# wiedehopf/readsb

Hardware: AMD Instinct MI355X
Metric: IQ Msamples/s demodulated (UC8 2.4 MSps stream, --fix), whole job (higher is better)
Workload: dtype u16

## Files before the change

### readsb_amd/csrc/api.cpp

```cpp
#include "ctx.h"

template <class Pred>
static void stage_wait(mgpu_ctx *c, std::unique_lock<std::mutex> &lk, Pred pred) {
    while (!pred()) {
        if (c->hot.load(std::memory_order_relaxed)) {
            lk.unlock();
            for (int i = 0; i < 32; ++i) __builtin_ia32_pause();
            sched_yield();
            lk.lock();
        } else {
            c->cv.wait(lk);
        }
    }
}

static hipError_t wait_event_spin(hipEvent_t ev) {
    for (unsigned spin = 0;; ++spin) {
        const hipError_t e = hipEventQuery(ev);
        if (e != hipErrorNotReady) return e;
        for (int k = 0; k < 128; ++k) __builtin_ia32_pause();
        if ((spin & 1023) == 1023) sched_yield();
    }
}
static hipError_t wait_stream_spin(hipStream_t s) {
// ... 19 lines not shown
void mgpu_config_defaults(struct mgpu_config *cfg) { config_defaults(cfg); }
void mgpu_config_defaults_abi(struct mgpu_config *cfg, uint32_t struct_bytes, uint32_t abi_version) {
    struct mgpu_config full;
    config_defaults(&full);
    full.abi_version = abi_version;
    std::memcpy(cfg, &full, struct_bytes < sizeof(full) ? struct_bytes : sizeof(full));
}
static void config_defaults(struct mgpu_config *cfg) {
    std::memset(cfg, 0, sizeof(*cfg));
    cfg->device = 0;
    cfg->format = MGPU_FMT_UC8;
    cfg->nfix_crc = 1;
    cfg->fixDF = 1;
    cfg->preamble_threshold = 58;
    cfg->buf_samples = 131072;
    cfg->trailing_samples = kTrailing;
    cfg->max_samples = 64ull * 131072;
    cfg->startup_time_ms = 0;
    cfg->abi_version = MGPU_ABI_VERSION;
}

uint32_t mgpu_abi_version(void) { return MGPU_ABI_VERSION; }

const char *mgpu_strerror(int code) {
    switch (code) {
        case MGPU_OK: return "ok";
        case MGPU_E_INVAL: return "invalid argument or state";
        case MGPU_E_NODEVICE: return "no usable HIP device (libmodes_gpu has no CPU fallback)";
        case MGPU_E_HIP: return "HIP runtime error";
        case MGPU_E_NOMEM: return "out of memory";
        case MGPU_E_OVERFLOW: return "device record pool overflow";
        case MGPU_E_CAPACITY: return "more samples than max_samples";
        case MGPU_E_EOF: return "stream already ended on a short buffer";
        default: return "unknown error";
    }
}

const char *mgpu_last_error(mgpu_ctx *ctx) { return ctx ? ctx->err.c_str() : ""; }

int mgpu_device_count(void) {
    int n = 0;
    if (hipGetDeviceCount(&n) != hipSuccess) return 0;
    return n;
}

static int alloc_slot(mgpu_ctx *c, Slot &sl) {
    const uint64_t n = c->chunk_samples;
    const uint64_t mag_len = (n + kTile - 1) / kTile * kTile + kTile + kHalo + 64;
    HIPCHK(c, hipMalloc(&sl.d_mag, mag_len * sizeof(uint16_t)));
    HIPCHK(c, hipMemsetAsync(sl.d_mag, 0, mag_len * sizeof(uint16_t), c->stream));
    HIPCHK(c, hipMalloc(&sl.d_pool, c->cap_pool * sizeof(PhaseRec)));
    HIPCHK(c, hipMalloc(&sl.d_unit_first, (c->cap_units * (size_t) (kUnit / 2048) + 1) * sizeof(uint32_t)));
    HIPCHK(c, hipMalloc(&sl.d_unit_count, (c->cap_units * (size_t) (kUnit / 2048) + 1) * sizeof(uint32_t)));
    HIPCHK(c, hipMalloc(&sl.d_unit_live, (c->cap_units + 2 + 3 * (c->cap_units / 4 + 2)) * sizeof(uint32_t)));
    sl.class_bytes = (mag_len / 32 + 64 + kUnit / 32) * sizeof(uint32_t);
    HIPCHK(c, hipMalloc(&sl.d_class_final, sl.class_bytes));
    HIPCHK(c, hipMalloc(&sl.d_cand, (c->cap_units * (size_t) kUnit + 64) * sizeof(uint16_t)));
    HIPCHK(c, hipMalloc(&sl.d_cand_count, (c->cap_units * (size_t) (kUnit / kSweepTile) + 1) * sizeof(uint32_t)));
    HIPCHK(c, hipMalloc(&sl.d_dealer, (size_t) 2 * kDealerCounters * kDealerStride * sizeof(uint32_t)));
    HIPCHK(c, hipMemsetAsync(sl.d_dealer, 0, (size_t) 2 * kDealerCounters * kDealerStride * sizeof(uint32_t), c->stream));
    HIPCHK(c, hipMalloc(&sl.d_sweep_part, ((size_t) kSweepGridMax * 4) * sizeof(uint32_t)));
    {
        const size_t nb = c->cap_buffers, words = CNT_NUM + 1 + 4 * nb + kAcLists;
        sl.scratch_bytes = words * sizeof(unsigned long long);
        HIPCHK(c, hipMalloc(&sl.d_scratch, sl.scratch_bytes));
        HIPCHK(c, hipMemsetAsync(sl.d_scratch, 0, sl.scratch_bytes, c->stream));
        HIPCHK(c, hipHostMalloc(&sl.h_scratch, sl.scratch_bytes));
        sl.d_counters = sl.d_scratch;
        sl.d_pool_used = (uint32_t *) (sl.d_scratch + CNT_NUM);
        sl.d_sum_level = sl.d_scratch + CNT_NUM + 1;
        sl.d_sum_power = sl.d_sum_level + nb;
        sl.d_fsum_level = (double *) (sl.d_sum_power + nb);
        sl.d_fsum_power = sl.d_fsum_level + nb;
        sl.h_counters = sl.h_scratch;
        sl.h_sums = sl.h_scratch + CNT_NUM + 1;
        sl.h_fsums = (double *) (sl.h_scratch + CNT_NUM + 1 + 2 * nb);
        if (c->cfg.format != MGPU_FMT_UC8) {
            HIPCHK(c, hipMalloc(&sl.d_fsx, 2 * nb * sizeof(double)));
            HIPCHK(c, hipHostMalloc(&sl.h_fsx, 2 * nb * sizeof(double)));
            HIPCHK(c, hipMemsetAsync(sl.d_fsx, 0, 2 * nb * sizeof(double), c->stream));
            sl.d_fsum_level = sl.d_fsx; sl.d_fsum_power = sl.d_fsx + nb; sl.h_fsums = sl.h_fsx;
        }
    }
    HIPCHK(c, hipMalloc(&sl.d_win, 8 * sizeof(unsigned long long)));
    HIPCHK(c, hipMalloc(&sl.d_win_part, kWinPartWords * sizeof(unsigned long long)));
    HIPCHK(c, hipMalloc(&sl.d_msg_pos, c->cap_msgs * sizeof(uint32_t)));
    HIPCHK(c, hipMalloc(&sl.d_msg_limit, c->cap_msgs * sizeof(uint32_t)));
    HIPCHK(c, hipMalloc(&sl.d_msg_len, c->cap_msgs * sizeof(uint16_t)));
    HIPCHK(c, hipMalloc(&sl.d_msg_skip, c->cap_msgs * sizeof(uint16_t)));
    HIPCHK(c, hipMalloc(&sl.d_msg_sig, c->cap_msgs * sizeof(unsigned long long)));
    {
        const size_t blob = c->cap_msgs * sizeof(Accepted) + c->cap_buffers * sizeof(BufferClock) + 64;
        HIPCHK(c, hipMalloc(&sl.d_blob, blob));
        HIPCHK(c, hipHostMalloc(&sl.h_blob, blob));
    }
    HIPCHK(c, hipMalloc(&sl.d_live, c->cap_pool * sizeof(PhaseRec)));
    HIPCHK(c, hipMalloc(&sl.d_live_sig, c->cap_pool * sizeof(unsigned long long)));
    HIPCHK(c, hipHostMalloc(&sl.h_live, c->cap_pool * sizeof(PhaseRec)));
    HIPCHK(c, hipHostMalloc(&sl.h_live_sig, c->cap_pool * sizeof(unsigned long long)));
    HIPCHK(c, hipEventCreateWithFlags(&sl.ev_window, hipEventDisableTiming));
    HIPCHK(c, hipEventCreateWithFlags(&sl.ev_scan, hipEventDisableTiming));
    HIPCHK(c, hipEventCreateWithFlags(&sl.ev_swept, hipEventDisableTiming));
    HIPCHK(c, hipEventCreateWithFlags(&sl.ev_h2d, hipEventDisableTiming));
    HIPCHK(c, hipEventCreateWithFlags(&sl.ev_pre, hipEventDisableTiming));
    HIPCHK(c, hipEventCreateWithFlags(&sl.ev_fsum, hipEventDisableTiming));
    HIPCHK(c, hipEventCreateWithFlags(&sl.ev_convdone, hipEventDisableTiming));
    HIPCHK(c, hipHostMalloc(&sl.h_win, 8 * sizeof(unsigned long long)));
    HIPCHK(c, hipHostMalloc(&sl.h_sig, c->cap_msgs * sizeof(unsigned long long)));
    HIPCHK(c, hipHostMalloc(&sl.h_msg_pos, c->cap_msgs * sizeof(uint32_t)));
    HIPCHK(c, hipHostMalloc(&sl.h_msg_limit, c->cap_msgs * sizeof(uint32_t)));
    HIPCHK(c, hipHostMalloc(&sl.h_msg_len, c->cap_msgs * sizeof(uint16_t)));
    HIPCHK(c, hipHostMalloc(&sl.h_msg_skip, c->cap_msgs * sizeof(uint16_t)));
    if (c->cfg.mode_ac) {
// ... 406 lines not shown
}

static int enqueue_sweep(mgpu_ctx *c, Slot &sl) {
    const mgpu_config &cfg = c->cfg;
    const uint64_t n = sl.n;
    const uint32_t nunits = (uint32_t) ((n + kUnit - 1) / kUnit);
    hipStream_t s = c->stream;
    SweepParams sp{};
    sp.mag = sl.d_mag; sp.n = n; sp.thr = sl.thr;
    sp.valid_long = c->valid_long; sp.valid_short = c->valid_short;
    sp.fix_df = (cfg.fixDF && cfg.nfix_crc) ? 1 : 0;
    sp.bit_syndrome = c->d_bit_syndrome; sp.parity = c->d_parity; sp.group_syndrome = c->d_group_syndrome;
    sp.tab_long = c->d_tab_long; sp.tab_short = c->d_tab_short; sp.n_long = c->n_long; sp.n_short = c->n_short;
    sp.pool = sl.d_pool; sp.pool_cap = (uint32_t) c->cap_pool; sp.pool_used = sl.d_pool_used;
    sp.unit_first = sl.d_unit_first; sp.unit_count = sl.d_unit_count; sp.nunits = nunits; sp.dealer = sl.d_dealer;
    sp.adder_bitmap = c->d_adder_bitmap; sp.counters = sl.d_counters;
    sp.cand = sl.d_cand; sp.cand_count = sl.d_cand_count; sp.sweep_part = sl.d_sweep_part;
    if (sl.fused_iq) {
        sp.iq = sl.fused_iq; sp.iq_format = (uint32_t) cfg.format; sp.tail = sl.fused_tail; sp.uc8_sym = c->d_uc8_folded + UC8_SYM_OFFSET; sp.mag_w = sl.d_mag;
        sp.sum_level = sl.d_sum_level; sp.sum_power = sl.d_sum_power;
        sp.buf_steps = cfg.buf_samples / (uint32_t) kSweepTile;
    }
#if MGPU_EXPERIMENTS
    sp.debug_stage = c->dbg_stage;
#endif
    {
        sl.sweep_blocks = launch_sweep(sp, s);
        if (sl.timed) HIPCHK(c, hipEventRecord(sl.ev[4], s));
        HIPCHK(c, hipEventRecord(sl.ev_swept, s));
        sl.swept_seq.store(sl.seq, std::memory_order_release);
        if (cfg.format != MGPU_FMT_UC8 && !cfg.mode_ac && !sl.have_mag && sl.fsum_iq) {
            const int rc = enqueue_fsum(c, sl, sl.fsum_iq, sl.ev_swept);
            if (rc != MGPU_OK) return rc;
        }
        sl.slice_blocks = launch_slice(sp, s);
    }
    if (sl.timed) HIPCHK(c, hipEventRecord(sl.ev[2], s));
    return MGPU_OK;
}

static int enqueue_post(mgpu_ctx *c, Slot &sl) {
    const uint64_t n = sl.n;
    const uint32_t nunits = (uint32_t) ((n + kUnit - 1) / kUnit);
    hipStream_t s = c->stream;

    PostSweepParams q{};
    q.pool = sl.d_pool; q.pool_cap = (uint32_t) c->cap_pool; q.variant = c->prescreen_variant; q.unit_first = sl.d_unit_first; q.first_count = sl.d_unit_count; q.nunits = nunits; q.chains_per_unit = (uint32_t) (kUnit / 2048); q.adder_bitmap = c->d_adder_bitmap;
    q.unit_live = sl.d_unit_live; q.block_live = sl.d_unit_live + c->cap_units + 2; q.live = sl.d_live; q.live_sig = sl.d_live_sig; q.counters = sl.d_counters;
    sl.sig_late = (c->sig_late && c->shard_mode == 0) || c->shard_mode == 3;
    q.mag = sl.sig_late ? nullptr : sl.d_mag;
    q.class_final = sl.d_class_final;
    q.class_words = (n + 31) / 32;
    q.dealer = sl.d_dealer;
    q.cand = sl.d_cand; q.cand_count = sl.d_cand_count;
    q.live_win = c->shard_mode == 2 ? sl.d_live_win : nullptr; q.n = n; q.thr = sl.thr; q.buf_len = c->cfg.buf_samples;
    q.d_scratch = sl.d_scratch; q.h_scratch = sl.h_scratch; q.scratch_words = (uint32_t) (sl.scratch_bytes / sizeof(unsigned long long));
    q.fin_part = q.block_live + c->cap_units / 4 + 2;
    q.slice_part = sl.d_sweep_part; q.slice_blocks = sl.slice_blocks;
    if (launch_prescreen(q, s, s, sl.ev_scan) != 0) { c->err = "event ordering of the pre-screen passes failed"; return MGPU_E_HIP; }
    if (sl.timed) HIPCHK(c, hipEventRecord(sl.ev[3], s));
    HIPCHK(c, hipEventRecord(sl.ev_done, s));
    return MGPU_OK;
}

static int enqueue_slot(mgpu_ctx *c, Slot &sl, const uint8_t *iq, hipEvent_t after_convert = nullptr) {
    int rc = enqueue_convert(c, sl, iq);
    const bool fsum_late = (c->cfg.format != MGPU_FMT_UC8 && !c->cfg.mode_ac && !sl.have_mag) || sweep_is_fused(c, sl);
    auto mark_read = [&]() -> int {
        if (sl.fsum_pending) {
            HIPCHK(c, hipEventRecord(sl.ev_convdone, c->stream));
            HIPCHK(c, hipStreamWaitEvent(c->stream_f, sl.ev_convdone, 0));
            HIPCHK(c, hipEventRecord(after_convert, c->stream_f));
        } else HIPCHK(c, hipEventRecord(after_convert, c->stream));
        return MGPU_OK;
    };
    if (rc == MGPU_OK && after_convert && !fsum_late) rc = mark_read();
    if (rc == MGPU_OK) rc = enqueue_sweep(c, sl);
    if (rc == MGPU_OK && after_convert && fsum_late) rc = mark_read();
    if (rc == MGPU_OK) rc = enqueue_post(c, sl);
    return rc;
}

static void unpin_records(mgpu_ctx *c, Slot &sl, HostJob &job, bool team) {
    const uint64_t nlive = job.nlive;
    job.recs.resize(nlive + 1);
    job.recs[nlive].pos = 0xFFFFFFFFu;
    if (!sl.sig_late) job.sig.resize(nlive);
    const int parts = team && nlive >= 65536 ? c->walk_threads : 1;
    auto copy = [&](int i) {
        const uint64_t lo = nlive * (uint64_t) i / parts, hi = nlive * (uint64_t) (i + 1) / parts;
        std::memcpy(job.recs.data() + lo, sl.h_live + lo, (hi - lo) * sizeof(PhaseRec));
        if (!sl.sig_late) std::memcpy(job.sig.data() + lo, sl.h_live_sig + lo, (hi - lo) * sizeof(unsigned long long));
    };
    if (parts > 1) c->walk_team.run(parts, copy); else copy(0);
    if (c->shard_mode == 2) job.win.assign(sl.h_live_win, sl.h_live_win + nlive);
    job.fetched = true;
}

static int fetch_records(mgpu_ctx *c, Slot &sl, HostJob &job) {
    const uint64_t nlive = job.nlive;
    if (nlive) {
        HIPCHK(c, hipMemcpyAsync(sl.h_live, sl.d_live, nlive * sizeof(PhaseRec), hipMemcpyDeviceToHost, c->stream_d2h));
        if (!sl.sig_late) HIPCHK(c, hipMemcpyAsync(sl.h_live_sig, sl.d_live_sig, nlive * sizeof(unsigned long long), hipMemcpyDeviceToHost, c->stream_d2h));
        if (c->shard_mode == 2) HIPCHK(c, hipMemcpyAsync(sl.h_live_win, sl.d_live_win, nlive * sizeof(unsigned long long), hipMemcpyDeviceToHost, c->stream_d2h));
        HIPCHK(c, wait_stream_spin(c->stream_d2h));
    }
    if (!c->dump_dir.empty()) {
        const char *dd = c->dump_dir.c_str();
        static int dumped = 0;
        if (!dumped++) {
            std::string base = std::string(dd) + "/walk_";
            FILE *f = fopen((base + "recs.bin").c_str(), "wb"); fwrite(sl.h_live, sizeof(PhaseRec), nlive, f); fclose(f);
            f = fopen((base + "sig.bin").c_str(), "wb"); fwrite(sl.h_live_sig, 8, nlive, f); fclose(f);
            f = fopen((base + "bufs.bin").c_str(), "wb"); fwrite(sl.buffers.data(), sizeof(BufferClock), sl.buffers.size(), f); fclose(f);
        }
    }
    unpin_records(c, sl, job, false);
    return MGPU_OK;
}

static int fetch_slot(mgpu_ctx *c, Slot &sl, HostJob &job) {
    HIPCHK(c, wait_event_spin(sl.ev_done));
    const double t_gpu_done = wall_ms();
    if (sl.h_counters[CNT_POOL_OVERFLOW]) {
        c->err = "record pool overflow: recreate the context with a larger record_pool_records";
        return MGPU_E_OVERFLOW;
    }
    float ms;
    if (sl.timed) {
        if (!sl.fused_iq && hipEventElapsedTime(&ms, sl.ev[0], sl.ev[1]) == hipSuccess) c->acc.convert_ms += ms;
        if (hipEventElapsedTime(&ms, sl.ev[1], sl.ev[4]) == hipSuccess) { c->acc.sweep_ms += ms; sweep_pace_feedback(ms * 1e3f, sl.n, sl.sweep_blocks, c->event_bracket_us, !sl.fused_iq ? 0 : c->cfg.format == MGPU_FMT_UC8 ? 1 : 2); }
        if (hipEventElapsedTime(&ms, sl.ev[4], sl.ev[2]) == hipSuccess) c->acc.slice_ms += ms;
        if (hipEventElapsedTime(&ms, sl.ev[2], sl.ev[3]) == hipSuccess) c->acc.prescreen_ms += ms;
        c->acc.n_timed_chunks += 1;
        if (sl.fused_iq) c->acc.sweep_fused_chunks += 1.0f;
    }
    const uint64_t nlive = sl.h_counters[CNT_LIVE_TOTAL];

    const double t_f0 = wall_ms();
    if (nlive > c->cap_pool) { c->err = "live record count beyond the pool"; return MGPU_E_OVERFLOW; }
    job.nlive = nlive;
    job.stream_pos = sl.stream_pos;
    job.fetched = job.from_device = false;
    job.sig_late = sl.sig_late;
    if ((c->device_walk != 1 || c->shard_mode != 0) && c->shard_mode != 1) { const int rc = fetch_records(c, sl, job); if (rc != MGPU_OK) return rc; }
    job.ac.clear();
    if (c->cfg.mode_ac && (!sl.have_mag || sl.have_noise)) {
        const unsigned long long *counts = sl.h_scratch + CNT_NUM + 1 + 4 * c->cap_buffers;
        const uint64_t cap_l = c->cap_ac / kAcLists;
        for (int l = 0; l < kAcLists; ++l) {
            if (counts[l] > cap_l) { c->err = "Mode A/C candidate buffer overflow"; return MGPU_E_OVERFLOW; }
            job.ac.insert(job.ac.end(), sl.h_ac + (size_t) l * cap_l, sl.h_ac + (size_t) l * cap_l + counts[l]);
        }
    }
    job.buffers = sl.buffers;
    job.given_mean_power = sl.given_mean_power;
    job.sums.assign(sl.h_sums, sl.h_sums + 2 * c->cap_buffers);
    job.fsum_idx = -1;
    if (sl.fsum_pending) {
        sl.fsum_pending = false;
        if (c->shard_mode == 0) job.fsum_idx = sl.fsum_idx;
        else {
            HIPCHK(c, wait_event_spin(c->fsum_ring[sl.fsum_idx].ev));
            std::memcpy(sl.h_fsums, c->fsum_ring[sl.fsum_idx].h, 2 * c->cap_buffers * sizeof(double));
        }
    }
    if (job.fsum_idx < 0) job.fsums.assign(sl.h_fsums, sl.h_fsums + 2 * c->cap_buffers);
    const unsigned long long *hc = sl.h_counters;
    if (!(c->shard_stream && job.stream_pos < c->shard_stream_own_first)) {
        c->feed_cand[0] += hc[CNT_CANDIDATES];
        for (int i = 0; i < 5; ++i) c->feed_cand[1 + i] += hc[CNT_PHASE0 + i];
        c->feed_cand[6] += hc[CNT_CLASS_COND];
        c->feed_cand[7] += hc[CNT_CLASS_UNCOND];
    }
    c->acc.n_candidates += hc[CNT_CANDIDATES];
    c->acc.n_records += hc[CNT_RECORDS];
    c->acc.n_live_records += nlive;
    c->acc.n_chunks += 1;
    c->acc.d2h_ms += (float) (wall_ms() - t_f0);
// ... 1152 lines not shown
```

### readsb_amd/csrc/ctx.h

```cpp
#pragma once
#include <hip/hip_runtime.h>
#include <pthread.h>
#include <dirent.h>
#include <sched.h>

#include <cctype>
#include <algorithm>
#include <atomic>
#include <functional>
#include <chrono>
#include <condition_variable>
#include <deque>
#include <mutex>
#include <thread>
#include <cmath>
#include <cstdio>
#include <cstdlib>
#include <cstring>
#include <limits>
#include <new>
#include <string>
#include <vector>

#include "../../include/modes_gpu.h"
// ... 56 lines not shown
  private:
    void work(uint32_t g, const std::function<void(int)> *fn, int n) {
        int done = 0;
        uint64_t t = ticket_.load(std::memory_order_acquire);
        for (;;) {
            if ((uint32_t) (t >> 32) != g || (int) (uint32_t) t >= n) break;
            if (!ticket_.compare_exchange_weak(t, t + 1, std::memory_order_acq_rel)) continue;
            (*fn)((int) (uint32_t) t);
            ++done;
            t = ticket_.load(std::memory_order_acquire);
        }
        if (done && pending_.fetch_sub(done, std::memory_order_acq_rel) == done) {
            std::lock_guard<std::mutex> lk(mu_);
            cv_done_.notify_all();
        }
    }
    void loop() {
        uint64_t seen = wake_.load(std::memory_order_acquire);
        for (;;) {
            for (int spin = 0; wake_.load(std::memory_order_acquire) == seen; ++spin) {
                __builtin_ia32_pause();
                if ((spin & 63) == 63) sched_yield();
                if (spin >= 4000 && !(hot_ && hot_->load(std::memory_order_relaxed))) break;
            }
            const std::function<void(int)> *fn;
            int n;
            uint32_t g;
            {
                std::unique_lock<std::mutex> lk(mu_);
                cv_work_.wait(lk, [&] { return quit_ || wake_.load(std::memory_order_acquire) != seen; });
                if (quit_) return;
                seen = wake_.load(std::memory_order_acquire);
                fn = fn_; n = ntasks_; g = gen_;
            }
            if (fn) work(g, fn, n);
        }
    }
    std::mutex mu_;
    std::condition_variable cv_work_, cv_done_;
    const std::function<void(int)> *fn_ = nullptr;
    int ntasks_ = 0;
    uint32_t gen_ = 0;
    std::atomic<uint64_t> ticket_{0}, wake_{0};
    std::atomic<int> pending_{0};
    const std::atomic<bool> *hot_ = nullptr;
    bool quit_ = false;
};

struct Slot {
    uint16_t *d_mag = nullptr;
    PhaseRec *d_pool = nullptr;
    uint32_t *d_dealer = nullptr;
    uint32_t *d_pool_used = nullptr, *d_unit_first = nullptr, *d_unit_count = nullptr, *d_unit_live = nullptr;
    uint32_t *d_class_final = nullptr, *d_cand_count = nullptr, *d_sweep_part = nullptr;
    uint16_t *d_cand = nullptr;
    size_t class_bytes = 0;
    unsigned long long *d_scratch = nullptr, *h_scratch = nullptr;
    size_t scratch_bytes = 0;
    unsigned long long *d_counters = nullptr, *d_sum_level = nullptr, *d_sum_power = nullptr, *d_win = nullptr, *d_msg_sig = nullptr;
    unsigned long long *d_win_part = nullptr;
    double *d_fsum_level = nullptr, *d_fsum_power = nullptr;
    uint32_t *d_msg_pos = nullptr, *d_msg_limit = nullptr;
    uint16_t *d_msg_len = nullptr, *d_msg_skip = nullptr;
    PhaseRec *d_live = nullptr;
    unsigned long long *d_live_sig = nullptr;
    unsigned long long *d_live_win = nullptr, *h_live_win = nullptr;
    PhaseRec *h_live = nullptr;
    unsigned long long *h_live_sig = nullptr;
    hipEvent_t ev_window = nullptr;
    bool window_pending = false;
    unsigned long long *h_counters = nullptr, *h_sums = nullptr, *h_win = nullptr, *h_sig = nullptr;
    double *h_fsums = nullptr;
    double *d_fsx = nullptr, *h_fsx = nullptr;
    uint32_t *h_msg_pos = nullptr, *h_msg_limit = nullptr;
    uint16_t *h_msg_len = nullptr, *h_msg_skip = nullptr;
    hipEvent_t ev_done = nullptr;
    hipEvent_t ev[5] = {};
    bool timed = false;
    uint32_t slice_blocks = 0;
    uint32_t sweep_blocks = 0;
    uint32_t *d_ac_noise = nullptr;
    AcCand *h_ac = nullptr;
    hipEvent_t ev_h2d = nullptr;
    hipEvent_t ev_pre = nullptr, ev_fsum = nullptr, ev_convdone = nullptr;
    bool fsum_pending = false;
    const uint8_t *fsum_iq = nullptr;
    int fsum_idx = -1;
    hipEvent_t ev_scan = nullptr;
    hipEvent_t ev_swept = nullptr;
    std::atomic<uint64_t> swept_seq{~0ull};
    const uint8_t *fused_iq = nullptr;
    const uint16_t *fused_tail = nullptr;
    uint64_t seq = 0;
    uint64_t n = 0, stream_pos = 0;
    uint8_t *d_wk_in = nullptr;
    void *d_wk_acc = nullptr;
    unsigned long long *d_wk_sig = nullptr;
    uint8_t *h_blob = nullptr, *d_blob = nullptr;
    bool sig_late = false;
    int feed = -1;
    int32_t thr = 58;
    bool have_mag = false, busy = false;
    bool have_noise = false;
    uint32_t given_noise = 0;
    std::vector<BufferClock> buffers;
    std::vector<double> given_mean_power;
// ... 228 lines not shown
```

### readsb_amd/csrc/kernels.h

```cpp
#pragma once
#ifndef MGPU_EXPERIMENTS
#define MGPU_EXPERIMENTS 0
#endif
#include <hip/hip_runtime.h>
#include <cstdint>

#include "../../include/modes_gpu.h"

namespace mgpu {

constexpr int kWinPartWords = 8192 * 8;
constexpr int kTrailing = 326;
constexpr int kTile = 4096;
constexpr int kHalo = 304;
constexpr int kTilesPerUnit = 2;
constexpr int kUnit = kTile * kTilesPerUnit;
constexpr int kBlock = 256;
constexpr int kSweepTile = 1024;
#ifndef MGPU_SL_WGS_PER_CU
#define MGPU_SL_WGS_PER_CU 4
#endif
constexpr int kSweepMaxBlocks = 256 * MGPU_SL_WGS_PER_CU;
constexpr int kSweepGridMax = 256 * 8;
constexpr int kDealerCounters = 64;
constexpr int kDealerStride = 64;
constexpr int kPoolChunkRecords = 256;
constexpr int kSweepMaxWaves = kSweepMaxBlocks * (kBlock / 64);
constexpr uint32_t kNone = 0xFFFFFFFFu;

enum : uint8_t {
    REC_ACCEPT_IF_UNKNOWN = 1,
    REC_ADDER = 2,
    REC_DFFIX = 4,
    REC_LONG = 8,
    REC_CORR_SHIFT = 4,
    REC_COND = 64,
};

struct PhaseRec {
    uint32_t pos;
    uint8_t phase;
    uint8_t flags;
    int16_t score_known;
    int16_t score_unknown;
    uint8_t fixbit0, fixbit1;
    uint32_t addr;
    uint8_t msg[14];
    uint16_t pad;
};
static_assert(sizeof(PhaseRec) == 32, "PhaseRec must be 32 bytes");
static_assert(sizeof(mgpu_msg) == 64 && sizeof(mgpu_fields) == 176, "C-ABI record sizes");

enum {
    CNT_CANDIDATES = 0,
    CNT_PHASE0 = 1,
    CNT_RECORDS = 6,
    CNT_POOL_OVERFLOW = 7,
    CNT_CLASS_COND = 8,
    CNT_CLASS_UNCOND = 9,
    CNT_DEBUG0 = 16,
    CNT_LIVE_TOTAL = 31,
    CNT_NUM = 32,
};

struct SweepParams {
    const uint16_t *mag;
    uint64_t n;
    int32_t thr;
    uint32_t valid_long;
    uint32_t valid_short;
    int32_t fix_df;
    const uint32_t *bit_syndrome;
    const uint64_t *parity;
    const uint32_t *group_syndrome;
    const uint64_t *tab_long;
    const uint64_t *tab_short;
    int32_t n_long, n_short;
    PhaseRec *pool;
    uint32_t pool_cap;
    uint32_t *pool_used;
    uint32_t *unit_first;
    uint32_t *unit_count;
    uint32_t *dealer;
    uint32_t nunits;
    uint16_t *cand;
    uint32_t *cand_count;
    uint32_t pace_recip;
    uint32_t *sweep_part;
    uint32_t *adder_bitmap;
    unsigned long long *counters;
    const uint8_t *iq;
    uint32_t iq_format;
    const uint16_t *tail;
    const uint16_t *uc8_sym;
    uint16_t *mag_w;
    unsigned long long *sum_level, *sum_power;
    uint32_t buf_steps;
#if MGPU_EXPERIMENTS
    int32_t debug_stage;
    unsigned long long *dbg_waves;
#endif
};

struct ConvertParams {
    const uint8_t *iq;
    uint16_t *mag;
    uint64_t n;
    uint32_t buf_samples;
    const uint16_t *tail;
    const uint16_t *uc8_folded;
    unsigned long long *sum_level;
    unsigned long long *sum_power;
    double *fsum_level;
    double *fsum_power;
};

void launch_convert(int format, const ConvertParams &p, hipStream_t s);
void launch_spin(unsigned us, unsigned blocks, unsigned long long *sink, hipStream_t s);
void launch_fsum_sc16(int format, const uint8_t *iq, uint64_t n, uint32_t buf_samples, double *fsum_level, double *fsum_power, int want_level,
                      hipStream_t s, int fresh = 0);
#if MGPU_EXPERIMENTS
size_t fsum_wide_scratch_bytes(uint64_t max_samples, uint32_t buf_samples);
void launch_fsum_sc16_wide(int format, const uint8_t *iq, const uint16_t *mag, uint64_t n, uint32_t buf_samples, double *fsum_level, double *fsum_power,
                           int want_level, void *scratch, hipStream_t s);
#endif
unsigned launch_sweep(const SweepParams &p, hipStream_t s);
void sweep_pace_feedback(float kernel_us, uint64_t n, unsigned blocks, float bracket_us, int fused = 0);
unsigned launch_slice(const SweepParams &p, hipStream_t s);
struct PostSweepParams {
    PhaseRec *pool;
    uint32_t pool_cap;
    uint32_t variant;
    const uint32_t *unit_first;
    const uint32_t *first_count;
    uint32_t chains_per_unit;
    uint32_t nunits;
    const uint32_t *adder_bitmap;
    uint32_t *unit_live;
    uint32_t *block_live;
    PhaseRec *live;
    const uint16_t *mag;
    unsigned long long *live_sig;
    unsigned long long *counters;
    uint32_t *class_final;
    uint64_t class_words;
    uint32_t *dealer;
    const uint16_t *cand; const uint32_t *cand_count;
    unsigned long long *live_win;
    uint64_t n; int32_t thr; uint32_t buf_len;
    unsigned long long *d_scratch, *h_scratch;
    uint32_t scratch_words;
    uint32_t *fin_part;
    const uint32_t *slice_part;
    uint32_t slice_blocks;
};
int launch_prescreen(const PostSweepParams &q, hipStream_t s, hipStream_t s_write, hipEvent_t ev_scan);
constexpr int kAcLists = 64;
struct AcCand {
    uint32_t pos;
    uint32_t f2_clock;
    uint32_t modeac;
};
void launch_modeac(const uint16_t *mag, uint64_t n, uint32_t buf_samples, int format, const unsigned long long *sum_level,
                   const unsigned long long *sum_power, const double *fsum_level, const double *fsum_power,
                   uint32_t *noise_level, AcCand *out, uint32_t cap, unsigned long long *list_counts ,
                   unsigned long long *counters, hipStream_t s);
void launch_modeac_scan(const uint16_t *mag, uint64_t n, uint32_t buf_samples, const uint32_t *noise_level, AcCand *out, uint32_t cap,
                        unsigned long long *list_counts, unsigned long long *counters, hipStream_t s);
void launch_decode_fields(const mgpu_msg *msgs, uint64_t n, mgpu_fields *out, const double *roll_tan, hipStream_t s);
void launch_beast_encode(const mgpu_msg *msgs, uint64_t n, uint16_t *meta, uint32_t *block_bytes, unsigned long long *block_off, uint8_t *out,
                         uint64_t cap, unsigned long long *total , hipStream_t s, const uint8_t *verdict = nullptr, int net_rule = 0,
                         uint32_t *block_def = nullptr, unsigned long long *block_def_off = nullptr, mgpu_deferred *deferred = nullptr, uint64_t def_cap = 0);
size_t gate_table_bytes();
size_t gate_scratch_bytes(uint64_t n);
void launch_track_gate(const mgpu_msg *msgs, const mgpu_fields *fields, uint64_t n, uint32_t buf_samples, void *table, void *scratch,
                       uint8_t *verdict, hipStream_t s);
void launch_signal_power(const uint16_t *mag, const uint32_t *pos, const uint16_t *len, uint32_t nmsg,
                         unsigned long long *out, hipStream_t s);
void launch_build_messages(const PhaseRec *live, const unsigned long long *live_sig, const unsigned long long *msg_sig, const void *d_acc,
                           const void *d_bufs, uint32_t nacc, mgpu_msg *out, hipStream_t s);
void launch_stage_blob(const void *h_src, void *d_dst, uint64_t bytes, hipStream_t s);

constexpr uint32_t kWkNoAdd = 0xffffffffu;
constexpr uint32_t kWkTouchedCap = 1u << 16;
constexpr int kWkCounts = 16;
constexpr int32_t kWkNoFlip = 0x7fffffff;
struct WalkIn {
    int64_t next_flip;
    uint32_t nbuf, n_active, n_inactive, acc_cap;
    uint32_t nlive, buf_len, pad[2];
};
static_assert(sizeof(WalkIn) == 40, "WalkIn");
constexpr uint32_t kWkInHead = 48;
struct WalkState {
    int32_t flip;
    uint32_t converged, iterations, bad;
    uint32_t n_touched[2];
    uint32_t cur, done;
};
// ... 34 lines not shown
```

### readsb_amd/csrc/kernels/prescreen.inc

```


__device__ __forceinline__ uint32_t write_unit_sequential(uint32_t u, const PhaseRec *pool, const uint32_t *unit_first, uint32_t cpu, uint32_t nunits,
                                                          uint32_t dst0, PhaseRec *live, const uint16_t *mag, unsigned long long *live_sig) {
    const int lane = lane_id();
    if (u >= nunits) return 0;
    uint32_t nlive = 0;
    uint32_t heads = kNone;
    if ((uint32_t) lane < cpu) heads = unit_first[u * cpu + (uint32_t) lane];
    for (uint32_t ch = 0; ch < cpu; ++ch) {
        uint32_t h = (uint32_t) __builtin_amdgcn_readlane((int) heads, (int) ch);
        while (h != kNone) {
            const uint32_t next = pool[h].addr;
            const uint64_t m = ((const unsigned long long *) &pool[h])[2];
            const bool ok = (m >> lane) & 1;
            uint32_t pos = 0, len = 0;
            if (ok) {
                const PhaseRec &r = pool[h + 1 + (uint32_t) lane];
                pos = r.pos;
                len = (r.msg[0] & 0x80) ? 268u : 134u;
                const uint32_t d = dst0 + nlive + __popcll(m & ((1ull << lane) - 1));
                const u32x4 *src = (const u32x4 *) &r;
                u32x4 *dd = (u32x4 *) &live[d];
                dd[0] = src[0]; dd[1] = src[1];
            }
// ... 143 lines not shown
            first = false;
            const uint32_t t0 = (uint32_t) __builtin_amdgcn_readlane((int) hd1.w, 0);
            base1 = base0 + t0;
            total = t0;
            if (CPU == 4) {
                const uint32_t t1 = (uint32_t) __builtin_amdgcn_readlane((int) hd1.w, 1), t2 = (uint32_t) __builtin_amdgcn_readlane((int) hd1.w, 2),
                               t3 = (uint32_t) __builtin_amdgcn_readlane((int) hd1.w, 3);
                base2 = base1 + t1; base3 = base2 + t2;
                total = t0 + t1 + t2 + t3;
            }
        }
#define MGPU_WR_LOAD(ch, base) \
        const uint32_t hc##ch = (uint32_t) __builtin_amdgcn_readlane((int) h, ch); \
        const uint64_t m##ch = (uint64_t) (uint32_t) __builtin_amdgcn_readlane((int) hd1.x, ch) | ((uint64_t) (uint32_t) __builtin_amdgcn_readlane((int) hd1.y, ch) << 32); \
        const bool ok##ch = hc##ch != kNone && ((m##ch >> lane) & 1); \
        const uint32_t d##ch = (base) + (uint32_t) __builtin_amdgcn_readlane((int) hd1.z, ch) + (uint32_t) __popcll(m##ch & lt_mask); \
        u32x4 a##ch = {0u, 0u, 0u, 0u}, b##ch = {0u, 0u, 0u, 0u}; \
        if (ok##ch) { const u32x4 *src = (const u32x4 *) &pool[hc##ch + 1u + (uint32_t) lane]; a##ch = src[0]; b##ch = src[1]; }
#define MGPU_WR_STORE(ch) \
        if (ok##ch) { u32x4 *dd = (u32x4 *) &live[d##ch]; dd[0] = a##ch; dd[1] = b##ch; }
        MGPU_WR_LOAD(0, base0)
        if (CPU == 4) {
            MGPU_WR_LOAD(1, base1) MGPU_WR_LOAD(2, base2) MGPU_WR_LOAD(3, base3)
            MGPU_WR_STORE(0) MGPU_WR_STORE(1) MGPU_WR_STORE(2) MGPU_WR_STORE(3)
        } else {
            MGPU_WR_STORE(0)
        }
#undef MGPU_WR_LOAD
#undef MGPU_WR_STORE
        WAVE_SYNC();
        if (h != kNone) h = hd0.w;
    }
    return total;
}

__global__ __launch_bounds__(kBlock) void k_count(PhaseRec *pool, uint32_t pool_cap, const uint32_t *unit_first, const uint32_t *first_count, uint32_t cpu, uint32_t nunits,
                                                  const uint32_t *bitmap, uint32_t *unit_live, uint32_t *block_live, uint32_t *final_bitmap,
                                                  unsigned long long *counters, uint32_t *part) {
    __shared__ uint32_t s_live[kBlock / WAVE], s_nc[kBlock / WAVE], s_nu[kBlock / WAVE];
    __shared__ __attribute__((aligned(16))) uint32_t s_cls[kBlock / WAVE][2 * (kUnit / 32)];
    const uint32_t wv = threadIdx.x >> 6, u = blockIdx.x * (kBlock / WAVE) + wv;
    uint32_t nlive, nc, nu;
    if (cpu == 4) nlive = count_unit_chains<4>(u, pool, pool_cap, unit_first, first_count, nunits, bitmap, counters, s_cls[wv], final_bitmap, nc, nu);
    else nlive = count_unit_chains<1>(u, pool, pool_cap, unit_first, nullptr, nunits, bitmap, counters, s_cls[wv], final_bitmap, nc, nu);
    if (lane_id() == 0) { s_live[wv] = nlive; s_nc[wv] = nc; s_nu[wv] = nu; if (u < nunits) unit_live[u] = nlive; }
    __syncthreads();
    if (threadIdx.x == 0) {
        block_live[blockIdx.x] = s_live[0] + s_live[1] + s_live[2] + s_live[3];
        part[2 * blockIdx.x] = s_nc[0] + s_nc[1] + s_nc[2] + s_nc[3];
        part[2 * blockIdx.x + 1] = s_nu[0] + s_nu[1] + s_nu[2] + s_nu[3];
    }
}

template <bool SIG>
__global__ __launch_bounds__(kBlock) void k_prescreen_write(PhaseRec *pool, const uint32_t *unit_first, uint32_t cpu, uint32_t nunits,
                                                            int by_chains, const uint32_t *unit_live, const uint32_t *block_live,
                                                            PhaseRec *live, const uint16_t *mag, unsigned long long *live_sig,
                                                            unsigned long long *counters, const uint32_t *fin_part, uint32_t nb_fin,
                                                            const uint32_t *slice_part, uint32_t slice_blocks) {
    __shared__ uint32_t s_part[kBlock / WAVE];
    if (blockIdx.x == 0 && slice_blocks) {
        unsigned long long a[5] = {0, 0, 0, 0, 0};
        for (uint32_t r = threadIdx.x; r < slice_blocks; r += kBlock) {
#pragma unroll
            for (int k = 0; k < 5; ++k) a[k] += slice_part[r * kSlPartWords + k];
        }
#pragma unroll
        for (int k = 0; k < 5; ++k) a[k] = wave_sum_u64(a[k]);
        if (lane_id() == 0) {
            if (a[0]) atomicAdd(&counters[CNT_RECORDS], a[0]);
            if (a[1]) atomicAdd(&counters[CNT_CANDIDATES], a[1]);
            if (a[2]) { atomicAdd(&counters[CNT_PHASE0 + 0], a[2]); atomicAdd(&counters[CNT_PHASE0 + 1], a[2]); }
            if (a[3]) { atomicAdd(&counters[CNT_PHASE0 + 2], a[3]); atomicAdd(&counters[CNT_PHASE0 + 3], a[3]); }
            if (a[4]) atomicAdd(&counters[CNT_PHASE0 + 4], a[4]);
        }
    }
    if (blockIdx.x == 0 && nb_fin) {
        unsigned long long a = 0, b = 0;
        for (uint32_t i = threadIdx.x; i < nb_fin; i += kBlock) { a += fin_part[2 * i]; b += fin_part[2 * i + 1]; }
        a = wave_sum_u64(a); b = wave_sum_u64(b);
        if (lane_id() == 0) {
            if (a) atomicAdd(&counters[CNT_CLASS_COND], a);
            if (b) atomicAdd(&counters[CNT_CLASS_UNCOND], b);
        }
    }
    uint32_t acc = 0;
    for (uint32_t i = threadIdx.x; i < blockIdx.x; i += kBlock) acc += block_live[i];
    acc = (uint32_t) wave_sum_u64(acc);
    const uint32_t wv = threadIdx.x >> 6;
    if (lane_id() == 0) s_part[wv] = acc;
    __syncthreads();
    uint32_t dst0 = s_part[0] + s_part[1] + s_part[2] + s_part[3];
    const uint32_t u = blockIdx.x * (kBlock / WAVE) + wv;
    for (uint32_t v = blockIdx.x * (kBlock / WAVE); v < u && v < nunits; ++v) dst0 += unit_live[v];
    uint32_t nlive;
    if (!SIG && by_chains && cpu == 4) nlive = write_unit_chains<4>(u, pool, unit_first, nunits, dst0, live);
    else if (!SIG && by_chains) nlive = write_unit_chains<1>(u, pool, unit_first, nunits, dst0, live);
    else nlive = write_unit_sequential(u, pool, unit_first, cpu, nunits, dst0, live, SIG ? mag : nullptr, SIG ? live_sig : nullptr);
    if (u == nunits - 1 && lane_id() == 0) counters[CNT_LIVE_TOTAL] = dst0 + nlive;
}

__global__ __launch_bounds__(kBlock) void k_publish(unsigned long long *d_scratch, unsigned long long *h_scratch, uint32_t nwords, uint32_t *dealer) {
    if (blockIdx.x == 0 && dealer && threadIdx.x < 2 * kDealerCounters) dealer[threadIdx.x * kDealerStride] = 0;
    for (uint32_t i = blockIdx.x * kBlock + threadIdx.x; i < nwords; i += gridDim.x * kBlock) {
        h_scratch[i] = d_scratch[i];
        d_scratch[i] = 0;
    }
}

#if MGPU_EXPERIMENTS
__global__ __launch_bounds__(kBlock) void k_prescreen_check(const PhaseRec *pool, const uint32_t *unit_first, uint32_t cpu, uint32_t nunits, const uint32_t *unit_live, unsigned long long *counters) {
    const uint32_t u = blockIdx.x * kBlock + threadIdx.x;
    if (u >= nunits) return;
    uint32_t all = 0;
    for (uint32_t ch = 0; ch < cpu; ++ch) {
        uint32_t h = unit_first[u * cpu + ch], run = 0, seg = 0;
        const uint32_t h0 = h;
        while (h != kNone) {
            const uint32_t *hw = (const uint32_t *) &pool[h];
            const uint64_t m = (uint64_t) hw[4] | ((uint64_t) hw[5] << 32);
            if (hw[6] != run && atomicAdd(&counters[CNT_DEBUG0], 1ull) < 8)
                printf("check: unit %u chain %u segment %u header %u: prefix %u, expected %u (cnt %u mask %llx next %u)\n", u, ch, seg, h, hw[6], run, hw[0], (unsigned long long) m, hw[3]);
            if (hw[0] < 64 && (m >> hw[0]) && atomicAdd(&counters[CNT_DEBUG0], 1ull) < 8)
                printf("check: unit %u chain %u segment %u header %u: mask %llx beyond cnt %u\n", u, ch, seg, h, (unsigned long long) m, hw[0]);
            run += (uint32_t) __popcll(m);
            h = hw[3];
            ++seg;
        }
        if (h0 != kNone && ((const uint32_t *) &pool[h0])[7] != run && atomicAdd(&counters[CNT_DEBUG0], 1ull) < 8)
            printf("check: unit %u chain %u first header %u: total %u, expected %u (%u segments)\n", u, ch, h0, ((const uint32_t *) &pool[h0])[7], run, seg);
        all += run;
    }
    if (all != unit_live[u] && atomicAdd(&counters[CNT_DEBUG0], 1ull) < 8) printf("check: unit %u: live %u, chains add up to %u\n", u, unit_live[u], all);
}
#endif

#if MGPU_EXPERIMENTS
__global__ __launch_bounds__(kBlock) void k_prescreen_check_live(const PhaseRec *pool, const uint32_t *unit_first, uint32_t cpu, uint32_t nunits, const uint32_t *unit_live, const PhaseRec *live, unsigned long long *counters) {
    const uint32_t u = blockIdx.x * kBlock + threadIdx.x;
    if (u >= nunits) return;
    uint32_t d = 0;
    for (uint32_t v = 0; v < u; ++v) d += unit_live[v];
    if (u == 0) printf("live: checked %u units\n", nunits);
    for (uint32_t ch = 0; ch < cpu; ++ch) {
        uint32_t h = unit_first[u * cpu + ch], seg = 0;
        while (h != kNone) {
            const uint32_t *hw = (const uint32_t *) &pool[h];
            const uint64_t m = (uint64_t) hw[4] | ((uint64_t) hw[5] << 32);
            for (uint32_t i = 0; i < hw[0]; ++i) {
                if (!((m >> i) & 1)) continue;
                const uint32_t *a = (const uint32_t *) &pool[h + 1 + i], *b = (const uint32_t *) &live[d];
                bool same = true;
                for (int k = 0; k < 8; ++k) same = same && a[k] == b[k];
                if (!same && atomicAdd(&counters[CNT_DEBUG0 + 1], 1ull) < 12)
                    printf("live: unit %u chain %u segment %u header %u record %u of %u -> live[%u]: pos %u addr %06x, found pos %u addr %06x (mask %llx prefix %u total7 %u)\n",
                           u, ch, seg, h, i, hw[0], d, a[0], a[3], b[0], b[3], (unsigned long long) m, hw[6], hw[7]);
                ++d;
            }
            h = hw[3];
            ++seg;
        }
    }
}
#endif

int launch_prescreen(const PostSweepParams &q, hipStream_t s, hipStream_t s_write, hipEvent_t ev_scan) {
    if (q.nunits == 0) return 0;
    if (q.chains_per_unit != 4 && q.chains_per_unit != 1) return -1;
    const unsigned nb_count = (q.nunits + 3) / 4;
    const unsigned nb_fin = nb_count;
    hipLaunchKernelGGL(k_count, dim3(nb_count), dim3(kBlock), 0, s, q.pool, q.pool_cap, q.unit_first, q.first_count, q.chains_per_unit, q.nunits, q.adder_bitmap,
                       q.unit_live, q.block_live, q.class_final, q.counters, q.fin_part);
#if MGPU_EXPERIMENTS
    if (q.variant & 4) hipLaunchKernelGGL(k_prescreen_check, dim3((q.nunits + kBlock - 1) / kBlock), dim3(kBlock), 0, s, q.pool, q.unit_first, q.chains_per_unit, q.nunits, q.unit_live, q.counters);
#endif
    if (s_write != s) {
        if (hipEventRecord(ev_scan, s) != hipSuccess || hipStreamWaitEvent(s_write, ev_scan, 0) != hipSuccess) return -1;
    }
#define MGPU_WRITE_ARGS dim3(nb_count), dim3(kBlock), 0, s_write, q.pool, q.unit_first, q.chains_per_unit, q.nunits, (q.variant & 2) ? 1 : 0, \
                        q.unit_live, q.block_live, q.live, q.mag, q.live_sig, q.counters, q.fin_part, nb_fin, q.slice_part, q.slice_blocks
    if (q.mag) hipLaunchKernelGGL((k_prescreen_write<true>), MGPU_WRITE_ARGS);
    else hipLaunchKernelGGL((k_prescreen_write<false>), MGPU_WRITE_ARGS);
#undef MGPU_WRITE_ARGS
#if MGPU_EXPERIMENTS
    if (q.variant & 4) hipLaunchKernelGGL(k_prescreen_check_live, dim3((q.nunits + kBlock - 1) / kBlock), dim3(kBlock), 0, s_write, q.pool, q.unit_first, q.chains_per_unit, q.nunits, q.unit_live, q.live, q.counters);
#endif
    if (q.live_win)
        launch_live_windows(q.mag, q.n, q.cand, q.cand_count, q.class_final, q.live, q.counters + CNT_LIVE_TOTAL, q.buf_len, q.live_win, s_write);
    unsigned pb = (q.scratch_words + kBlock - 1) / kBlock;
    if (pb > 64) pb = 64;
    hipLaunchKernelGGL(k_publish, dim3(pb), dim3(kBlock), 0, s_write, q.d_scratch, q.h_scratch, q.scratch_words, q.dealer);
    return 0;
}
```

Before: 462,400.

## Fuse prescreen count and write into one persistent kernel with decoupled look-back scan

Adds a persistent k_prescreen_fused kernel that hands out tickets of units from a dealer counter, counts live records per unit, and computes output offsets with a decoupled look-back prefix scan. It then writes the live records in the same kernel, replacing the separate k_count and k_prescreen_write launches. The goal is to cut one launch and the global round trip of per-unit counts. It adds epoch-tagged look-back state, a stall counter and an error path. The path only runs when prescreen variant bit 8 is set, which may not be the default.

After: 439,100. 0.95x the previous value.

```diff
diff --git a/readsb_amd/csrc/api.cpp b/readsb_amd/csrc/api.cpp
--- a/readsb_amd/csrc/api.cpp
+++ b/readsb_amd/csrc/api.cpp
@@ -95,13 +95,15 @@
     HIPCHK(c, hipMalloc(&sl.d_pool, c->cap_pool * sizeof(PhaseRec)));
     HIPCHK(c, hipMalloc(&sl.d_unit_first, (c->cap_units * (size_t) (kUnit / 2048) + 1) * sizeof(uint32_t)));
     HIPCHK(c, hipMalloc(&sl.d_unit_count, (c->cap_units * (size_t) (kUnit / 2048) + 1) * sizeof(uint32_t)));
-    HIPCHK(c, hipMalloc(&sl.d_unit_live, (c->cap_units + 2 + 3 * (c->cap_units / 4 + 2)) * sizeof(uint32_t)));
+    sl.lookback_at = (c->cap_units + 2 + 3 * (c->cap_units / 4 + 2) + 1) / 2 * 2;
+    HIPCHK(c, hipMalloc(&sl.d_unit_live, (sl.lookback_at + 8 * (c->cap_units / 4 + 2)) * sizeof(uint32_t)));
+    HIPCHK(c, hipMemsetAsync(sl.d_unit_live, 0, (sl.lookback_at + 8 * (c->cap_units / 4 + 2)) * sizeof(uint32_t), c->stream));
     sl.class_bytes = (mag_len / 32 + 64 + kUnit / 32) * sizeof(uint32_t);
     HIPCHK(c, hipMalloc(&sl.d_class_final, sl.class_bytes));
     HIPCHK(c, hipMalloc(&sl.d_cand, (c->cap_units * (size_t) kUnit + 64) * sizeof(uint16_t)));
     HIPCHK(c, hipMalloc(&sl.d_cand_count, (c->cap_units * (size_t) (kUnit / kSweepTile) + 1) * sizeof(uint32_t)));
-    HIPCHK(c, hipMalloc(&sl.d_dealer, (size_t) 2 * kDealerCounters * kDealerStride * sizeof(uint32_t)));
-    HIPCHK(c, hipMemsetAsync(sl.d_dealer, 0, (size_t) 2 * kDealerCounters * kDealerStride * sizeof(uint32_t), c->stream));
+    HIPCHK(c, hipMalloc(&sl.d_dealer, (size_t) kDealerWords * sizeof(uint32_t)));
+    HIPCHK(c, hipMemsetAsync(sl.d_dealer, 0, (size_t) kDealerWords * sizeof(uint32_t), c->stream));
     HIPCHK(c, hipMalloc(&sl.d_sweep_part, ((size_t) kSweepGridMax * 4) * sizeof(uint32_t)));
     {
         const size_t nb = c->cap_buffers, words = CNT_NUM + 1 + 4 * nb + kAcLists;
@@ -614,6 +616,12 @@
     q.class_final = sl.d_class_final;
     q.class_words = (n + 31) / 32;
     q.dealer = sl.d_dealer;
+    q.lookback = (unsigned long long *) (sl.d_unit_live + sl.lookback_at);
+    if (++sl.prescreen_epoch >= (1u << 30)) {
+        HIPCHK(c, hipMemsetAsync(q.lookback, 0, (size_t) 4 * (c->cap_units / 4 + 2) * sizeof(unsigned long long), s));
+        sl.prescreen_epoch = 1;
+    }
+    q.epoch = sl.prescreen_epoch;
     q.cand = sl.d_cand; q.cand_count = sl.d_cand_count;
     q.live_win = c->shard_mode == 2 ? sl.d_live_win : nullptr; q.n = n; q.thr = sl.thr; q.buf_len = c->cfg.buf_samples;
     q.d_scratch = sl.d_scratch; q.h_scratch = sl.h_scratch; q.scratch_words = (uint32_t) (sl.scratch_bytes / sizeof(unsigned long long));
@@ -687,6 +695,10 @@
     if (sl.h_counters[CNT_POOL_OVERFLOW]) {
         c->err = "record pool overflow: recreate the context with a larger record_pool_records";
         return MGPU_E_OVERFLOW;
+    }
+    if (sl.h_counters[CNT_PRESCREEN_STALL]) {
+        c->err = "the pre-screen's look-back gave up waiting for an earlier ticket";
+        return MGPU_E_HIP;
     }
     float ms;
     if (sl.timed) {
diff --git a/readsb_amd/csrc/ctx.h b/readsb_amd/csrc/ctx.h
--- a/readsb_amd/csrc/ctx.h
+++ b/readsb_amd/csrc/ctx.h
@@ -132,6 +132,8 @@
     PhaseRec *d_pool = nullptr;
     uint32_t *d_dealer = nullptr;
     uint32_t *d_pool_used = nullptr, *d_unit_first = nullptr, *d_unit_count = nullptr, *d_unit_live = nullptr;
+    size_t lookback_at = 0;
+    uint32_t prescreen_epoch = 0;
     uint32_t *d_class_final = nullptr, *d_cand_count = nullptr, *d_sweep_part = nullptr;
     uint16_t *d_cand = nullptr;
     size_t class_bytes = 0;
diff --git a/readsb_amd/csrc/kernels.h b/readsb_amd/csrc/kernels.h
--- a/readsb_amd/csrc/kernels.h
+++ b/readsb_amd/csrc/kernels.h
@@ -24,6 +24,12 @@
 constexpr int kSweepGridMax = 256 * 8;
 constexpr int kDealerCounters = 64;
 constexpr int kDealerStride = 64;
+constexpr int kDealerWords = (2 * kDealerCounters + 1) * kDealerStride;
+#ifndef MGPU_FUSED_BATCH
+#define MGPU_FUSED_BATCH 4
+#endif
+constexpr int kFusedBatch = MGPU_FUSED_BATCH;
+constexpr int kFusedTicketUnits = kFusedBatch * (kBlock / 64);
 constexpr int kPoolChunkRecords = 256;
 constexpr int kSweepMaxWaves = kSweepMaxBlocks * (kBlock / 64);
 constexpr uint32_t kNone = 0xFFFFFFFFu;
@@ -58,6 +64,7 @@
     CNT_POOL_OVERFLOW = 7,
     CNT_CLASS_COND = 8,
     CNT_CLASS_UNCOND = 9,
+    CNT_PRESCREEN_STALL = 10,
     CNT_DEBUG0 = 16,
     CNT_LIVE_TOTAL = 31,
     CNT_NUM = 32,
@@ -145,6 +152,8 @@
     uint32_t *class_final;
     uint64_t class_words;
     uint32_t *dealer;
+    unsigned long long *lookback;
+    uint32_t epoch;
     const uint16_t *cand; const uint32_t *cand_count;
     unsigned long long *live_win;
     uint64_t n; int32_t thr; uint32_t buf_len;
diff --git a/readsb_amd/csrc/kernels/prescreen.inc b/readsb_amd/csrc/kernels/prescreen.inc
--- a/readsb_amd/csrc/kernels/prescreen.inc
+++ b/readsb_amd/csrc/kernels/prescreen.inc
@@ -219,6 +219,23 @@
     }
 }
 
+__device__ __forceinline__ void fold_slice_part(const uint32_t *slice_part, uint32_t slice_blocks, unsigned long long *counters) {
+    unsigned long long a[5] = {0, 0, 0, 0, 0};
+    for (uint32_t r = threadIdx.x; r < slice_blocks; r += kBlock) {
+#pragma unroll
+        for (int k = 0; k < 5; ++k) a[k] += slice_part[r * kSlPartWords + k];
+    }
+#pragma unroll
+    for (int k = 0; k < 5; ++k) a[k] = wave_sum_u64(a[k]);
+    if (lane_id() == 0) {
+        if (a[0]) atomicAdd(&counters[CNT_RECORDS], a[0]);
+        if (a[1]) atomicAdd(&counters[CNT_CANDIDATES], a[1]);
+        if (a[2]) { atomicAdd(&counters[CNT_PHASE0 + 0], a[2]); atomicAdd(&counters[CNT_PHASE0 + 1], a[2]); }
+        if (a[3]) { atomicAdd(&counters[CNT_PHASE0 + 2], a[3]); atomicAdd(&counters[CNT_PHASE0 + 3], a[3]); }
+        if (a[4]) atomicAdd(&counters[CNT_PHASE0 + 4], a[4]);
+    }
+}
+
 template <bool SIG>
 __global__ __launch_bounds__(kBlock) void k_prescreen_write(PhaseRec *pool, const uint32_t *unit_first, uint32_t cpu, uint32_t nunits,
                                                             int by_chains, const uint32_t *unit_live, const uint32_t *block_live,
@@ -226,22 +243,7 @@
                                                             unsigned long long *counters, const uint32_t *fin_part, uint32_t nb_fin,
                                                             const uint32_t *slice_part, uint32_t slice_blocks) {
     __shared__ uint32_t s_part[kBlock / WAVE];
-    if (blockIdx.x == 0 && slice_blocks) {
-        unsigned long long a[5] = {0, 0, 0, 0, 0};
-        for (uint32_t r = threadIdx.x; r < slice_blocks; r += kBlock) {
-#pragma unroll
-            for (int k = 0; k < 5; ++k) a[k] += slice_part[r * kSlPartWords + k];
-        }
-#pragma unroll
-        for (int k = 0; k < 5; ++k) a[k] = wave_sum_u64(a[k]);
-        if (lane_id() == 0) {
-            if (a[0]) atomicAdd(&counters[CNT_RECORDS], a[0]);
-            if (a[1]) atomicAdd(&counters[CNT_CANDIDATES], a[1]);
-            if (a[2]) { atomicAdd(&counters[CNT_PHASE0 + 0], a[2]); atomicAdd(&counters[CNT_PHASE0 + 1], a[2]); }
-            if (a[3]) { atomicAdd(&counters[CNT_PHASE0 + 2], a[3]); atomicAdd(&counters[CNT_PHASE0 + 3], a[3]); }
-            if (a[4]) atomicAdd(&counters[CNT_PHASE0 + 4], a[4]);
-        }
-    }
+    if (blockIdx.x == 0 && slice_blocks) fold_slice_part(slice_part, slice_blocks, counters);
     if (blockIdx.x == 0 && nb_fin) {
         unsigned long long a = 0, b = 0;
         for (uint32_t i = threadIdx.x; i < nb_fin; i += kBlock) { a += fin_part[2 * i]; b += fin_part[2 * i + 1]; }
@@ -267,8 +269,140 @@
     if (u == nunits - 1 && lane_id() == 0) counters[CNT_LIVE_TOTAL] = dst0 + nlive;
 }
 
+constexpr uint32_t kLbAggregate = 1, kLbInclusive = 2, kLbFailed = 3;
+constexpr uint32_t kLbMaxPolls = 1u << 15;
+constexpr int kLbWindows = 4;
+constexpr int kLbStride = 4;
+
+__device__ __forceinline__ unsigned long long lb_word(uint32_t epoch, uint32_t status, uint32_t value) {
+    return ((unsigned long long) epoch << 34) | ((unsigned long long) status << 32) | value;
+}
+
+__device__ __forceinline__ bool lookback_exclusive(const unsigned long long *lb, uint32_t t, uint32_t epoch, uint32_t &excl) {
+    const int lane = lane_id();
+    int hi = (int) t;
+    uint32_t sum = 0, polls = 0;
+    while (hi > 0) {
+        unsigned long long w[kLbWindows];
+#pragma unroll
+        for (int k = 0; k < kLbWindows; ++k) {
+            const int i = hi - 1 - k * WAVE - lane;
+            w[k] = i >= 0 ? __hip_atomic_load(&lb[(size_t) kLbStride * (size_t) i], __ATOMIC_RELAXED, __HIP_MEMORY_SCOPE_AGENT) : 0ull;
+        }
+        bool done = false, stuck = false;
+#pragma unroll
+        for (int k = 0; k < kLbWindows; ++k) {
+            if (done || stuck || hi <= 0) continue;
+            const bool in = hi - 1 - lane >= 0;
+            const uint32_t st = (in && (uint32_t) (w[k] >> 34) == epoch) ? (uint32_t) (w[k] >> 32) & 3u : 0u;
+            const uint64_t need = __ballot(in), ready = __ballot(st != 0), inc = __ballot(st == kLbInclusive), bad = __ballot(st == kLbFailed);
+            if (bad) return false;
+            const uint64_t upto = inc ? (((inc & (0 - inc)) << 1) - 1) & need : need;
+            if ((ready & upto) != upto) { stuck = true; continue; }
+            sum += (uint32_t) wave_sum_u64(((upto >> lane) & 1) ? (uint32_t) w[k] : 0u);
+            if (inc) done = true; else hi -= WAVE;
+        }
+        if (done) break;
+        if (stuck) {
+            if (++polls > kLbMaxPolls) return false;
+            __builtin_amdgcn_s_sleep(2);
+        }
+    }
+    excl = sum;
+    return true;
+}
+
+__global__ __launch_bounds__(kBlock, 5) void k_prescreen_fused(PhaseRec *pool, uint32_t pool_cap, const uint32_t *unit_first, const uint32_t *first_count, uint32_t nunits,
+                                                               const uint32_t *bitmap, uint32_t *unit_live, uint32_t *final_bitmap, PhaseRec *live,
+                                                               unsigned long long *counters, const uint32_t *slice_part, uint32_t slice_blocks,
+                                                               uint32_t *ticket_counter, unsigned long long *lb, uint32_t epoch) {
+    constexpr int kWaves = kBlock / WAVE, kB = kFusedBatch;
+    static_assert(kWaves == 4, "a group = four units, one per wave");
+    __shared__ uint32_t s_live[kB][kWaves], s_nc[kWaves], s_nu[kWaves], s_ticket, s_excl, s_fail;
+    __shared__ __attribute__((aligned(16))) uint32_t s_cls[kWaves][2 * (kUnit / 32)];
+    const uint32_t tid = threadIdx.x, wv = tid >> 6;
+    const int lane = lane_id();
+    const uint32_t ntickets = (nunits + kFusedTicketUnits - 1) / kFusedTicketUnits;
+    if (blockIdx.x == gridDim.x - 1 && slice_blocks) fold_slice_part(slice_part, slice_blocks, counters);
+    const uint32_t deal_zero = deal_opaque_zero();
+    uint32_t next = 0;
+    if (tid == 0) next = deal_ask(ticket_counter, deal_zero);
+    for (;;) {
+        if (tid == 0) s_ticket = next;
+        __syncthreads();
+        const uint32_t t = s_ticket;
+        if (t >= ntickets) break;
+        if (tid == 0) next = deal_ask(ticket_counter, deal_zero);
+        const uint32_t u0 = t * (uint32_t) kFusedTicketUnits + wv;
+        uint32_t nc = 0, nu = 0;
+#pragma unroll 1
+        for (int k = 0; k < kB; ++k) {
+            const uint32_t u = u0 + (uint32_t) (k * kWaves);
+            uint32_t c, uc;
+            const uint32_t nlive = count_unit_chains<4>(u, pool, pool_cap, unit_first, first_count, nunits, bitmap, counters, s_cls[wv], final_bitmap, c, uc);
+            nc += c; nu += uc;
+            if (lane == 0) { s_live[k][wv] = nlive; if (u < nunits) unit_live[u] = nlive; }
+        }
+        if (lane == 0) { s_nc[wv] = nc; s_nu[wv] = nu; }
+        __syncthreads();
+        uint32_t agg = 0, before = 0;
+#pragma unroll
+        for (int k = 0; k < kB; ++k) {
+#pragma unroll
+            for (int v = 0; v < kWaves; ++v) { agg += s_live[k][v]; if (k == 0 && (uint32_t) v < wv) before += s_live[k][v]; }
+        }
+        if (wv == 0) {
+            unsigned long long *const w = lb + (size_t) kLbStride * t;
+            if (lane == 0) {
+                __hip_atomic_store(&w[0], lb_word(epoch, t ? kLbAggregate : kLbInclusive, agg), __ATOMIC_RELAXED, __HIP_MEMORY_SCOPE_AGENT);
+                __hip_atomic_store(&w[1], ((unsigned long long) epoch << 32) | (s_nc[0] + s_nc[1] + s_nc[2] + s_nc[3]), __ATOMIC_RELAXED, __HIP_MEMORY_SCOPE_AGENT);
+                __hip_atomic_store(&w[2], ((unsigned long long) epoch << 32) | (s_nu[0] + s_nu[1] + s_nu[2] + s_nu[3]), __ATOMIC_RELAXED, __HIP_MEMORY_SCOPE_AGENT);
+            }
+            uint32_t excl = 0;
+            const bool ok = t == 0 || lookback_exclusive(lb, t, epoch, excl);
+            if (lane == 0) {
+                if (t) __hip_atomic_store(&w[0], ok ? lb_word(epoch, kLbInclusive, excl + agg) : lb_word(epoch, kLbFailed, 0), __ATOMIC_RELAXED, __HIP_MEMORY_SCOPE_AGENT);
+                s_excl = excl; s_fail = ok ? 0u : 1u;
+                if (!ok) atomicAdd(&counters[CNT_PRESCREEN_STALL], 1ull);
+            }
+        }
+        __syncthreads();
+        if (s_fail) return;
+        uint32_t dst0 = s_excl + before;
+#pragma unroll 1
+        for (int k = 0; k < kB; ++k) {
+            write_unit_chains<4>(u0 + (uint32_t) (k * kWaves), pool, unit_first, nunits, dst0, live);
+            if (k + 1 < kB)
+                for (int v = 0; v < kWaves; ++v) dst0 += (uint32_t) v >= wv ? s_live[k][v] : s_live[k + 1][v];
+        }
+        if (t == ntickets - 1) {
+            unsigned long long a = 0, b = 0;
+            bool ok = true;
+            for (uint32_t i = tid; i < 2 * ntickets; i += kBlock) {
+                const unsigned long long *const wp = &lb[(size_t) kLbStride * (i >> 1) + 1 + (i & 1)];
+                unsigned long long w = 0;
+                uint32_t polls = 0;
+                for (;;) {
+                    w = __hip_atomic_load(wp, __ATOMIC_RELAXED, __HIP_MEMORY_SCOPE_AGENT);
+                    if ((uint32_t) (w >> 32) == epoch) break;
+                    if (++polls > kLbMaxPolls) { ok = false; w = 0; break; }
+                    __builtin_amdgcn_s_sleep(2);
+                }
+                if (i & 1) b += (uint32_t) w; else a += (uint32_t) w;
+            }
+            a = wave_sum_u64(a); b = wave_sum_u64(b);
+            if (__ballot(!ok) && lane == 0) atomicAdd(&counters[CNT_PRESCREEN_STALL], 1ull);
+            if (lane == 0) {
+                if (a) atomicAdd(&counters[CNT_CLASS_COND], a);
+                if (b) atomicAdd(&counters[CNT_CLASS_UNCOND], b);
+            }
+            if (tid == 0) counters[CNT_LIVE_TOTAL] = s_excl + agg;
+        }
+    }
+}
+
 __global__ __launch_bounds__(kBlock) void k_publish(unsigned long long *d_scratch, unsigned long long *h_scratch, uint32_t nwords, uint32_t *dealer) {
-    if (blockIdx.x == 0 && dealer && threadIdx.x < 2 * kDealerCounters) dealer[threadIdx.x * kDealerStride] = 0;
+    if (blockIdx.x == 0 && dealer && threadIdx.x < kDealerWords / kDealerStride) dealer[threadIdx.x * kDealerStride] = 0;
     for (uint32_t i = blockIdx.x * kBlock + threadIdx.x; i < nwords; i += gridDim.x * kBlock) {
         h_scratch[i] = d_scratch[i];
         d_scratch[i] = 0;
@@ -336,6 +470,27 @@
     if (q.chains_per_unit != 4 && q.chains_per_unit != 1) return -1;
     const unsigned nb_count = (q.nunits + 3) / 4;
     const unsigned nb_fin = nb_count;
+    if ((q.variant & 8) && !q.mag && !q.live_win && q.chains_per_unit == 4 && q.dealer && q.lookback && s_write == s) {
+        static std::atomic<unsigned> resident_of[64];
+        int dev = 0;
+        (void) hipGetDevice(&dev);
+        unsigned resident = resident_of[dev & 63].load(std::memory_order_relaxed);
+        if (!resident) { resident = resident_grid((const void *) k_prescreen_fused, 0, 256u * 8u); resident_of[dev & 63].store(resident, std::memory_order_relaxed); }
+        const unsigned ntickets = (q.nunits + kFusedTicketUnits - 1) / kFusedTicketUnits;
+        hipLaunchKernelGGL(k_prescreen_fused, dim3(ntickets < resident ? ntickets : resident), dim3(kBlock), 0, s, q.pool, q.pool_cap, q.unit_first, q.first_count, q.nunits,
+                           q.adder_bitmap, q.unit_live, q.class_final, q.live, q.counters, q.slice_part, q.slice_blocks,
+                           q.dealer + (size_t) 2 * kDealerCounters * kDealerStride, q.lookback, q.epoch);
+#if MGPU_EXPERIMENTS
+        if (q.variant & 4) {
+            hipLaunchKernelGGL(k_prescreen_check, dim3((q.nunits + kBlock - 1) / kBlock), dim3(kBlock), 0, s, q.pool, q.unit_first, q.chains_per_unit, q.nunits, q.unit_live, q.counters);
+            hipLaunchKernelGGL(k_prescreen_check_live, dim3((q.nunits + kBlock - 1) / kBlock), dim3(kBlock), 0, s, q.pool, q.unit_first, q.chains_per_unit, q.nunits, q.unit_live, q.live, q.counters);
+        }
+#endif
+        unsigned pb = (q.scratch_words + kBlock - 1) / kBlock;
+        if (pb > 64) pb = 64;
+        hipLaunchKernelGGL(k_publish, dim3(pb), dim3(kBlock), 0, s, q.d_scratch, q.h_scratch, q.scratch_words, q.dealer);
+        return 0;
+    }
     hipLaunchKernelGGL(k_count, dim3(nb_count), dim3(kBlock), 0, s, q.pool, q.pool_cap, q.unit_first, q.first_count, q.chains_per_unit, q.nunits, q.adder_bitmap,
                        q.unit_live, q.block_live, q.class_final, q.counters, q.fin_part);
 #if MGPU_EXPERIMENTS
```
